# shamim-hussain/egt

Hardware: AMD Instinct MI355X
Metric: graphs/sec EGT fwd+bwd, ZINC-500K padded N=64 (higher is better)
Workload: dtype f32; 1 GPU; zinc500k_n64: attention-block stack (h,e,mask)->(h',e') x Ly, fwd+bwd + param grads; scope=stack, graphs_per_gpu=128, global_batch=128, N=64, Dh=64, De=64, H=8, d=8, Ly=10, parallelism=dp1, grad_allreduce_bytes=740480, backend=none (single process), flat_grad_adopted=True, flat_grad_bound=True, collective_in_graph=False

## Files before the change

### egt_amd/_lib.py

```python
from __future__ import annotations

import ctypes as C
import os

_HERE = os.path.dirname(os.path.abspath(__file__))
LIB_PATH = os.environ.get("EGT_AMD_LIB") or os.path.join(_HERE, "lib", "libegt_amd.so")

ABI_VERSION = 4
EGT_OK = 0
EGT_E_NULL, EGT_E_SHAPE, EGT_E_DTYPE, EGT_E_FLAGS, EGT_E_HIP, EGT_E_WORKSPACE, EGT_E_RCCL = -1, -2, -3, -4, -5, -6, -7
EGT_F32 = 0
EGT_BF16 = 1
F_EDGE_INPUT, F_GATE_INPUT, F_ATTN_MASK, F_SCALE_DEGREE = 0x001, 0x002, 0x004, 0x008
F_SCALER_LINEAR, F_TRAINING, F_CLIP = 0x010, 0x020, 0x040
ATTN_WS_SHARED = 0x1
EP_LAYERNORM, EP_GATES = 0x1, 0x2
ACT_NONE, ACT_LRELU, ACT_RELU, ACT_ELU = 0, 1, 2, 3
BF_GATE, BF_ATTN_MASK, BF_TRAINING, BF_CLIP, BF_NO_EDGE_LN, BF_SEED_DEVICE = 0x1, 0x2, 0x4, 0x8, 0x10, 0x20


class AttnDesc(C.Structure):
    _fields_ = [("B", C.c_int32), ("N", C.c_int32), ("H", C.c_int32), ("d", C.c_int32),
                ("dtype", C.c_int32), ("flags", C.c_uint32),
                ("clip_lo", C.c_float), ("clip_hi", C.c_float),
# ... 94 lines not shown
    "egt_dp_allreduce": (C.c_int, [_VP, C.c_size_t, C.c_int32, _VP]),
    "egt_dp_world": (C.c_int, []),
    "egt_dp_rank": (C.c_int, []),
    "egt_dp_finalize": (C.c_int, []),
    "egt_prof_enable": (C.c_int, [C.c_int]),
    "egt_prof_filter": (C.c_int, [C.c_char_p]),
    "egt_prof_stride": (C.c_int, [C.c_int]),
    "egt_prof_read": (C.c_int, [C.c_char_p, C.POINTER(C.c_int64), C.POINTER(C.c_double)]),
    "egt_prof_names": (C.c_int, [C.c_char_p, C.c_size_t]),
    "egt_prof_collect_graph": (C.c_int, [C.c_int]),
    "egt_prof_forget_graphs": (C.c_int, []),
}
_OPTIONAL_PROTOS = {
    "egt_block_supported": (C.c_int, [C.POINTER(BlockDesc)]),
    "egt_block_bwd_kernel": (C.c_char_p, [C.POINTER(BlockDesc)]),
    "egt_block_saved_bytes": (C.c_size_t, [C.POINTER(BlockDesc)]),
    "egt_block_workspace_bytes": (C.c_size_t, [C.POINTER(BlockDesc)]),
    "egt_block_fwd": (C.c_int, [C.POINTER(BlockDesc), C.POINTER(BlockParams)] + [_VP] * 10),
    "egt_block_bwd": (C.c_int, [C.POINTER(BlockDesc), C.POINTER(BlockParams)] + [_VP] * 10
                      + [C.POINTER(BlockParams)] + [_VP] * 2),
    "egt_stack_saved_bytes": (C.c_size_t, [C.POINTER(BlockDesc), C.c_int32]),
    "egt_stack_workspace_bytes": (C.c_size_t, [C.POINTER(BlockDesc), C.c_int32]),
    "egt_stack_fwd": (C.c_int, [C.POINTER(BlockDesc), C.c_int32, C.POINTER(BlockParams)] + [_VP] * 9),
    "egt_stack_bwd": (C.c_int, [C.POINTER(BlockDesc), C.c_int32, C.POINTER(BlockParams)] + [_VP] * 9
                      + [C.POINTER(BlockParams)] + [_VP] * 2),
    "egt_pair_supported": (C.c_int, [C.POINTER(BlockDesc)]),
    "egt_pair_workspace_bytes": (C.c_size_t, [C.POINTER(BlockDesc)]),
    "egt_pair_fwd": (C.c_int, [C.POINTER(BlockDesc), C.POINTER(BlockParams)] + [_VP] * 8),
    "egt_pair_bwd": (C.c_int, [C.POINTER(BlockDesc), C.POINTER(BlockParams)] + [_VP] * 9
                     + [C.POINTER(BlockParams)] + [_VP] * 2),
# ... 49 lines not shown
```

### egt_amd/csrc/egt_block.hip

```cpp
#include "egt_common.h"

#include <stdlib.h>
#include <string.h>
#include <vector>

#include "egt_block.h"
#include "egt_tile.h"

#include "egt_block_dev.h"
#include "egt_dma.h"

#include "egt_block_fwd.h"
#include "egt_block_bwd.h"



struct EgtBlockEnv {
  bool no_narrow_fwd, no_narrow_bwd;
  int bwd_mm;
  int bwd_tl, fwd_rows;
  int nrw_fwd_waves, nrw_bwd_waves, nrw_fwd_half;
};
static bool env_flag_raw(const char* name) {
  const char* v = getenv(name);
// ... 56 lines not shown

struct BlockPlan {
  bool ml;
  bool full;
  FwdKernel fwd;
  EgtLaunch fl;
  int fwd_nw;
  bool fwd_half;
  bool kvl;
  bool epi_ok;
  int RGF;
  BwdKernel bwd;
  EgtLaunch bl;
  int bwd_nw;
  int mm;
  int TL, NLR, nwg_bwd, EP;
  size_t v_att, stats, qkvp, pw_sv, wfrag_sv, saved_total;
  size_t dvp, dqp, dkvp, dqp_sz, dkvp_sz, common_total;
  size_t pw, epart, spart, sbo, wpart, ered, dqkv, dhbuf, layer_total;
};

template <int DE>
static BlockPlan plan_for(const egt_block_desc* d, bool ml) {
  using GG = Geo<DE>;
  const EgtBlockEnv& E = block_env();
  const int B = d->B, N = d->N, cus = egt_device_cus();
  const int groups = (N + BWD_TL - 1) / BWD_TL;
  BlockPlan P{};
  P.ml = ml;
  P.full = (N % 16) == 0;
// ... 29 lines not shown
  P.epi_ok = P.fwd != FwdKernel::tile || P.kvl;

  if (E.bwd_tl >= 4 && E.bwd_tl <= BWD_TL) P.TL = E.bwd_tl;
  else if (DE != 8) {
    const int g = tg > groups ? tg : groups;
    P.TL = (N + g - 1) / g;
  } else if (B * groups <= cus) {
    P.TL = BWD_TL;
    if (N > 8)
      for (int tl = 8; tl < BWD_TL; ++tl)
        if (B * ((N + tl - 1) / tl) <= cus) { P.TL = tl; break; }
  } else P.TL = (N + groups - 1) / groups;
  P.NLR = (N + P.TL - 1) / P.TL;
  P.nwg_bwd = B * P.NLR;
  P.EP = GG::EP;
  if (DE == 8 && !ml && !E.no_narrow_bwd) {
    P.bwd = BwdKernel::narrow;
    P.bwd_nw = E.nrw_bwd_waves == 8 || (E.nrw_bwd_waves != 4 && P.nwg_bwd <= cus && N >= 64) ? 8 : 4;
    P.bl = {P.nwg_bwd, 64 * P.bwd_nw, egt_narrow_bwd_lds(P.bwd_nw)};
  } else if (DE <= 16 && !ml) {
    constexpr int PWR = V4R_RR * (2 * GG::TILE_FLOATS + 256 + 192);
    P.bwd = BwdKernel::v4r;
    P.bl = {P.nwg_bwd, 256,
            ((size_t)(4 * PWR > BWD_PRO_WS ? 4 * PWR : BWD_PRO_WS) + (size_t)BWD_TL * QD_LD + 3 * GG::TILES * 256 + 3 * 2048 + 4) * 4};
  } else if (DE >= 32 && !ml && d->dtype != EGT_BF16) {
    P.bwd = BwdKernel::v5;
    P.mm = E.bwd_mm;
    P.bl = {P.nwg_bwd, 256, ((size_t)V5_AREA(DE) + (size_t)BWD_TL * QD_LD + 3 * ((GG::TILES + 1) / 2) * 512 + 4) * 4};
  } else {
    constexpr int PW = 3 * GG::TILE_FLOATS + 256 + 192;
    P.bwd = BwdKernel::v4;
    P.bl = {P.nwg_bwd, 256,
            ((size_t)(4 * PW > BWD_PRO_WS ? 4 * PW : BWD_PRO_WS) + (size_t)BWD_TL * QD_LD + 3 * ((GG::TILES + 1) / 2) * 512) * 4};
  }

  const size_t rows = (size_t)B * N;
  const int Dh = d->d * d->H;
  size_t o = 0;
  P.v_att = o; o += al(rows * Dh);
  P.stats = o; o += al(rows * BH * 4);
  P.qkvp = o; o += al(rows * QKVP);
  P.pw_sv = o; o += al((size_t)GG::DEP * 16 + 16);
// ... 36 lines not shown
  DISPATCH_BDE(d->De, return plan_for<DE>(d, ml));
}

static bool host_rand_mask(const egt_block_desc* d, const uint8_t* rm) {
  return rm && (d->flags & EGT_BF_TRAINING) && d->random_mask_prob > 0.0f;
}
static bool mask_tensor(const egt_block_desc* d, const uint8_t* rm) {
  return (d->flags & EGT_BF_ATTN_MASK) || host_rand_mask(d, rm);
}

static void bind_ws(const BlockPlan& P, BlockArgs& a, float* wc, float* wl, int parity = 0) {
  a.dvp = wc + P.dvp; a.dqp = wc + P.dqp + parity * P.dqp_sz; a.dkvp = wc + P.dkvp + parity * P.dkvp_sz;
  a.epart = wl + P.epart; a.spart = wl + P.spart; a.sbo = wl + P.sbo; a.wpart = wl + P.wpart;
  a.spart_n = a.sbo_n = a.B * ((a.N + NODE_RC - 1) / NODE_RC);
  a.ered = wl + P.ered; a.dqkv_sv = wl + P.dqkv;
  a.TL = P.TL; a.NLR = P.NLR; a.NQP = 1;
  a.xcd = 1;
}

extern "C" const char* egt_block_bwd_kernel(const egt_block_desc* d) {
  if (block_check(d, false)) return nullptr;
  return g_bwd_kernel_name[(int)plan_block(d, mask_tensor(d, nullptr)).bwd];
}

extern "C" size_t egt_block_saved_bytes(const egt_block_desc* d) {
  if (block_check(d, false)) return 0;
  return plan_block(d, mask_tensor(d, nullptr)).saved_total * sizeof(float);
}
extern "C" size_t egt_block_workspace_bytes(const egt_block_desc* d) {
  if (block_check(d, false)) return 0;
  const BlockPlan P = plan_block(d, mask_tensor(d, nullptr));
// ... 128 lines not shown
  static_assert(DE % 16 == 0 || DE == 8, "edge widths of the pair kernels");
  const bool pro = fuse;
  a.pro = 0;
  if (pro) {
    a.pro = top ? 1 : 2;
    a.sbo_n = P.nwg_bwd;
    if (!top) {
      a.up_h = above->h; a.up_nm_g = above->nm_g; a.up_Wqkv = above->Wqkv; a.up_wfrag = above->wfrag; a.up_dh_out = above->dh_out;
      a.up_dqp = above->dqp; a.up_dkvp = above->dkvp; a.up_dqkv_sv = above->dqkv_sv; a.up_spart = above->spart;
      above->spart_n = P.nwg_bwd;
    }
    if (a.prep) egt_node_launch_prep(&a, 1, st);
  } else if (top) {
    egt_node_launch_bwd(a, &a, false, st);
  }
  a.NQP = (a.N + 15) / 16;
  a.guard = 0;
  switch (P.bwd) {
    case BwdKernel::narrow: egt_narrow_launch_bwd(a, P.bwd_nw, P.bl, st); break;
    case BwdKernel::v4r:
      if constexpr (DE <= 16) {
        if (a.bf16) egt_launch_planned<k_block_bwd_v4r<DE, true, V4R_RR>>("k_block_bwd", P.bl, st, a);
        else egt_launch_planned<k_block_bwd_v4r<DE, false, V4R_RR>>("k_block_bwd", P.bl, st, a);
      }
      break;
    case BwdKernel::v5:
      if constexpr (DE >= 32) launch_v5<DE>(a, P, st);
      break;
    case BwdKernel::v4: if (a.bf16) launch_v4<DE, true>(a, P, st); else launch_v4<DE, false>(a, P, st); break;
  }
  if (!pro) egt_node_launch_bwd(a, below, true, st);
// ... 183 lines not shown
```

### egt_amd/csrc/egt_block_bwd.h

```cpp
#pragma once
#ifndef EGT_NT_BWD_E
#define EGT_NT_BWD_E true
#endif
#ifndef EGT_NT_BWD_DY
#define EGT_NT_BWD_DY false
#endif
#ifndef EGT_NT_BWD_ST
#define EGT_NT_BWD_ST false
#endif

template <int DE, bool ML, bool BF, bool RAG>
__global__ void __launch_bounds__(256, 2) k_block_bwd_v4(BlockArgs a) {
  seed_from_device(a);
  using G = Geo<DE>;
  typedef typename EdgeT<BF>::type ET;
  const ET* e_in = reinterpret_cast<const ET*>(a.e);
  ET* e_o = reinterpret_cast<ET*>(a.e_out);
  const ET* dey_in = reinterpret_cast<const ET*>(a.de_out);
  ET* dex_o = reinterpret_cast<ET*>(a.de);
  (void)e_in; (void)e_o; (void)dey_in; (void)dex_o;
  extern __shared__ __attribute__((aligned(16))) float sm[];
  const int lane = threadIdx.x & 63, wave = threadIdx.x >> 6;
  const int p = lane & 15, q = lane >> 4;
  const int N = a.N, TL = a.TL;
// ... 261 lines not shown
  if (p == 0) {
#pragma unroll
    for (int r = 0; r < 4; ++r) ep[G::DEP * 16 + 4 * q + r] = ssum[r];
  }
  __syncthreads();
  float* out = a.epart + (size_t)wg * G::EP;
  for (int i = threadIdx.x; i < G::EP; i += 256)
    out[i] = (sm[i] + sm[G::EP + i]) + (sm[2 * G::EP + i] + sm[3 * G::EP + i]);
}

#ifndef V5_BALANCE
#define V5_BALANCE 1
#endif
#define V5_AREA(DE_) ((4 * (3 * Geo<DE_>::TILE_FLOATS + 448) > 4 * Geo<DE_>::TILE_FLOATS + BWD_PRO_WS) \
                          ? 4 * (3 * Geo<DE_>::TILE_FLOATS + 448) : 4 * Geo<DE_>::TILE_FLOATS + BWD_PRO_WS)
template <int DE, int MM, bool RAG>
__global__ void __launch_bounds__(256, 2) k_block_bwd_v5(BlockArgs a) {
  seed_from_device(a);
#define PSTAMP(i) do {} while (0)
  constexpr bool SPLIT = MM == EGT_MM_BF16X3;
  constexpr int NS = (Geo<DE>::TILES + 1) / 2;
  (void)SPLIT; (void)NS;
  using G = Geo<DE>;
  const float* e_in = a.e;
  const float* dey_in = a.de_out;
  float* dex_o = a.de;
  extern __shared__ __attribute__((aligned(16))) float sm[];
  const int lane = threadIdx.x & 63, wave = __builtin_amdgcn_readfirstlane(threadIdx.x >> 6);
  const int p = lane & 15, q = lane >> 4;
  const int N = a.N, TL = a.TL;
// ... 15 lines not shown
  static_assert(4 * PW == 4 * G::TILE_FLOATS + 4 * PW2 && AREA >= 4 * PW && AREA >= 4 * G::TILE_FLOATS + BWD_PRO_WS, "tile area");
  float* pro_ws = sm + 4 * G::TILE_FLOATS;
  float* qd = sm + AREA;
  float* wsA = qd + TL * QD_LD;
  float* wsB = wsA + WSLAB;
  float* wsD = wsB + WSLAB;
  volatile int* pflag = reinterpret_cast<volatile int*>(wsD + WSLAB);
  if (threadIdx.x < 4) pflag[threadIdx.x] = 0;
  const unsigned et_lds = __builtin_amdgcn_readfirstlane((unsigned)(size_t)et0);
  const unsigned off0 = dma_lane_offset<DE>(lane);
  const int ntile = RAG ? (N + 15) / 16 : N / 16;
  const bool balance = RAG && V5_BALANCE && ntile >= 3 && (ntile & 3) != 0;
  const int T_ = ntile * nl;
  const int t0 = balance ? (wave * T_) >> 2 : 0, t1 = balance ? ((wave + 1) * T_) >> 2 : 0;
  const bool have = balance ? t1 > t0 : wave < ntile;
  const int mt_first = balance ? t0 / nl : wave, mt_last = balance ? (t1 - 1) / nl : ntile - 1, mt_step = balance ? 1 : 4;
  const int r0_first = balance ? t0 - mt_first * nl : 0;
  float Kf[16], Vf[16];
  int kmv = 1;
#define V5_TILE_START(MT_, ROW_)                                                                                    \
  do {                                                                                                              \
    const int m0_ = (MT_) * 16, kv_ = RAG ? min(16, N - m0_) : 16;                                                  \
    if (RAG && kv_ < 16) tile_dma_ragged<DE>(et_lds, e_in + (((size_t)b * N + l_begin + (ROW_)) * N + m0_) * DE, lane, kv_); \
    else tile_dma<DE, EGT_NT_BWD_E>(et_lds, e_in + (((size_t)b * N + l_begin + (ROW_)) * N + m0_) * DE, off0);      \
    const size_t rowm_ = (size_t)b * N + (RAG ? min(m0_ + p, N - 1) : m0_ + p);                                     \
    const float4* kp_ = reinterpret_cast<const float4*>(a.qkvp + rowm_ * QKVP + 64 + q * 16);                       \
    const float4* vp_ = reinterpret_cast<const float4*>(a.qkvp + rowm_ * QKVP + 128 + q * 16);                      \
    _Pragma("unroll") for (int i = 0; i < 4; ++i) {                                                                 \
      const float4 kv4 = kp_[i], vv4 = vp_[i];                                                                      \
      Kf[4*i] = kv4.x; Kf[4*i+1] = kv4.y; Kf[4*i+2] = kv4.z; Kf[4*i+3] = kv4.w;                                     \
// ... 99 lines not shown
    float dKa[16], dVa[16];
#pragma unroll
    for (int i = 0; i < 16; ++i) { dKa[i] = 0.f; dVa[i] = 0.f; }
    asm volatile("" : "+v"(kmv));
    const float kadd = kmv == 0 ? -EGT_NEG : 0.0f;
    const int l_first = l_begin + r0, l_stop = l_begin + r1;
    for (int l = l_first; l < l_stop; ++l) {
      const int li = l - l_begin;
      const int lj = l - l_first;
      const size_t rowl = (size_t)b * N + l;
      const size_t pair0 = rowl * N + m0;
      float* et = et0 + (lj & 1) * estr;
      MaskRegs mr{make_float2(1.f, 1.f), 0};
      TileRegs<DE> td;
      tile_gload<DE, EGT_NT_BWD_DY>(td, dey_in + pair0 * DE, lane, kv);
      if (lj == 0) vm_wait<(G::NF4 + 63) / 64>(); else vm_wait<2 * ((G::NF4 + 63) / 64) + 1>();
      SCHED_FENCE();
      float rstd;
      v4f acc = {c2r[0], c2r[1], c2r[2], c2r[3]};
      {
        float4 x[G::TILES];
#pragma unroll
        for (int t = 0; t < G::TILES; ++t) x[t] = frag_read<DE>(et, p, q, t);
        rstd = ln_frags<DE>(x, q, a.ln_eps, (a.flags & EGT_BF_NO_EDGE_LN) == 0);
        if constexpr (MM != 0) {
#pragma unroll
          for (int t = 0; t < G::TILES; ++t) frag_write<DE>(et, p, q, t, x[t]);
          v4f xv[G::TILES];
          Bf8 xh[NS], xl[NS];
#pragma unroll
          for (int t = 0; t < G::TILES; ++t) xv[t] = (v4f){x[t].x, x[t].y, x[t].z, x[t].w};
// ... 102 lines not shown
      {
        const float* qr = qd + li * QD_LD;
        const float4* qp = reinterpret_cast<const float4*>(qr + q * 16);
        const float4* dp = reinterpret_cast<const float4*>(qr + 64 + q * 16);
        float dq[16];
#pragma unroll
        for (int i = 0; i < 4; ++i) {
          const float4 u = qp[i], v = dp[i];
          dKa[4*i]   = fmaf(dA[0], u.x, dKa[4*i]);   dKa[4*i+1] = fmaf(dA[1], u.y, dKa[4*i+1]);
          dKa[4*i+2] = fmaf(dA[0], u.z, dKa[4*i+2]); dKa[4*i+3] = fmaf(dA[1], u.w, dKa[4*i+3]);
          dVa[4*i]   = fmaf(at[0], v.x, dVa[4*i]);   dVa[4*i+1] = fmaf(at[1], v.y, dVa[4*i+1]);
          dVa[4*i+2] = fmaf(at[0], v.z, dVa[4*i+2]); dVa[4*i+3] = fmaf(at[1], v.w, dVa[4*i+3]);
        }
#pragma unroll
        for (int k = 0; k < 8; ++k) { dq[2 * k] = dA[0] * Kf[2 * k]; dq[2 * k + 1] = dA[1] * Kf[2 * k + 1]; }
        a.dqp[(((size_t)b * ntile + mt) * N + l) * 64 + lane] = reduce16_keep_own(dq, p);
      }
      SCHED_FENCE();
      if (!(a.guard & 1))
      {
        float bT[4], bR[4];
#pragma unroll
        for (int s = 0; s < 4; ++s) {
          bT[s] = sc1[(q + 4 * s) * 16 + p];
          bR[s] = (p < 9) ? sc2[(q + 4 * s) * 12 + p] : 0.f;
        }
        {
          const int lb = 64 * q + 4 * ((p >> 2) ^ q) + (p & 3);
          const float* eb = et + lb;
          const float* db = dt + lb;
#pragma unroll
// ... 93 lines not shown
#pragma unroll
  for (int r = 0; r < 4; ++r) ssum[r] = row_sum16(ssum[r]);
  __syncthreads();
  float* ep = sm + wave * G::EP;
#pragma unroll
  for (int t = 0; t < G::TILES; ++t)
#pragma unroll
    for (int r = 0; r < 4; ++r) {
      ep[(16 * t + 4 * q + r) * 16 + p] = accT[t][r];
      ep[G::DEP * 16 + 16 + (16 * t + 4 * q + r) * 16 + p] = accR[t][r];
    }
  if (p == 0) {
#pragma unroll
    for (int r = 0; r < 4; ++r) ep[G::DEP * 16 + 4 * q + r] = ssum[r];
  }
  __syncthreads();
  float* out = a.epart + (size_t)wg * G::EP;
  for (int i = threadIdx.x; i < G::EP; i += 256)
    out[i] = (sm[i] + sm[G::EP + i]) + (sm[2 * G::EP + i] + sm[3 * G::EP + i]);
}

template <int DE, bool BF, int R>
__global__ void __launch_bounds__(256, 2) k_block_bwd_v4r(BlockArgs a) {
  seed_from_device(a);
  using G = Geo<DE>;
  typedef typename EdgeT<BF>::type ET;
  const ET* e_in = reinterpret_cast<const ET*>(a.e);
  const ET* dey_in = reinterpret_cast<const ET*>(a.de_out);
  ET* dex_o = reinterpret_cast<ET*>(a.de);
  extern __shared__ __attribute__((aligned(16))) float sm[];
  const int lane = threadIdx.x & 63, wave = threadIdx.x >> 6;
  const int p = lane & 15, q = lane >> 4;
  const int N = a.N, TL = a.TL;
  const int wg = a.xcd ? egt_xcd_remap(blockIdx.x, gridDim.x) : (int)blockIdx.x;
// ... 321 lines not shown
```

### egt_amd/csrc/egt_node.hip

```cpp
#include <stdlib.h>

#include "egt_block.h"

#define LDP 4

__device__ __forceinline__ float sum16(float v) { return row_sum16(v); }

__device__ __forceinline__ v4f mm_xw(const float* xs, int ld, const float* W, int ldw,
                                     int K, int p, int q, bool colok, v4f acc) {
#pragma unroll 4
  for (int t = 0; t < K; t += 4) {
    const float bv = colok ? W[(size_t)(t + q) * ldw + p] : 0.f;
    acc = MFMA(xs[p * ld + t + q], bv, acc);
  }
  return acc;
}
__device__ __forceinline__ v4f mm_xwt(const float* xs, int ld, const float* W, int ldw,
                                      int K, int p, int q, bool colok, v4f acc) {
#pragma unroll 4
  for (int t = 0; t < K; t += 4) {
    const float bv = colok ? W[(size_t)p * ldw + t + q] : 0.f;
    acc = MFMA(xs[p * ld + t + q], bv, acc);
  }
  return acc;
// ... 309 lines not shown
            a.h_out[o] = acc[r] + a.h[o];
          }
        }
      }
    }
  }
}

struct NodeBwdArgs {
  const float *wq_a, *wo_a;
  int wq_al, wo_al;
  const float *dv_Wo, *dv_v_att, *dv_dh_src;
  float *dv_stats, *dv_dvp, *dv_sbo;
};

template <bool PRE, bool DV, int NP>
__global__ void __launch_bounds__(512, 2) k_node_bwd(BlockArgs a, NodeBwdArgs x) {
  extern __shared__ __attribute__((aligned(16))) float sm[];
  const int NCH = (a.N + NODE_RC - 1) / NODE_RC;
  if ((int)blockIdx.x == a.B * NCH) { prep_device(a, sm); return; }
  const int Dh = a.Dh, N = a.N, b = blockIdx.x / NCH, chunk = blockIdx.x % NCH, t = threadIdx.x, D3 = 3 * Dh;
  const int ld = Dh + LDP, ld3 = D3 + LDP, SP = D3 + 2 * Dh;
  const int lane = t & 63, wave = __builtin_amdgcn_readfirstlane(t >> 6), p = lane & 15, q = lane >> 4, NW = blockDim.x >> 6;
  float* xs = sm;
  float* dls = xs + NODE_RC * ld;
  float* dhs = dls + NODE_RC * ld;
  float* vs = dhs + NODE_RC * ld;
  float* rs = vs + NODE_RC * ld;
  float* dlp = rs + NODE_RC;
  float* wo = dlp + 4 * NODE_RC * 8;
  float* dqs = wo + Dh * ld;
// ... 27 lines not shown
    }
    const int U = nrp * 48;
#pragma unroll
    for (int u = 0; u < 3; ++u) {
      const int i = t + u * 512, r = i / 48, pos4 = (i % 48) * 4, sx = pos4 >> 6;
      const bool ok = i < U && r < nr;
      const int rc = ok ? r : 0;
      float4 acc4 = make_float4(0.f, 0.f, 0.f, 0.f);
      const int np = sx == 0 ? a.NQP : a.NLR;
      const float* base = sx == 0 ? a.dqp + ((size_t)b * a.NQP * N + r0 + rc) * 64 + pos4
                                  : a.dkvp + (((size_t)b * a.NLR * N + r0 + rc) * 2 + (sx - 1)) * 64 + (pos4 & 63);
      const size_t pstride = sx == 0 ? (size_t)N * 64 : (size_t)N * 128;
      if (NP > 0) {
#pragma unroll
        for (int pi = 0; pi < NP; ++pi) {
          const float4 w = *reinterpret_cast<const float4*>(base + pi * pstride);
          acc4.x += w.x; acc4.y += w.y; acc4.z += w.z; acc4.w += w.w;
        }
      } else {
        const int npmax = max(a.NQP, a.NLR);
#pragma unroll 4
        for (int pi = 0; pi < npmax; ++pi) {
          const float4 w = *reinterpret_cast<const float4*>(base + min(pi, np - 1) * pstride);
          const float f = pi < np ? 1.0f : 0.0f;
          acc4.x = fmaf(w.x, f, acc4.x); acc4.y = fmaf(w.y, f, acc4.y);
          acc4.z = fmaf(w.z, f, acc4.z); acc4.w = fmaf(w.w, f, acc4.w);
        }
      }
      gq[u] = sel4(ok, acc4);
    }
  } else {
    stg_issue_rows(sX, x.dv_dh_src + row0 * Dh, Dh, nr, nrp);
// ... 137 lines not shown
    __syncthreads();
    for (int i = t; i < nr * 8; i += blockDim.x) {
      float dl = 0.f;
      for (int it = 0; it < nit; ++it) dl += dlp[it * NODE_RC * 8 + i];
      x.dv_stats[(row0 * BH + i) * 4 + 2] = dl;
    }
    if (a.DK < 8) {
      for (int i = t; i < nr * 64; i += blockDim.x)
        if ((((i & 63) >> 1) & 7) >= a.DK) x.dv_dvp[row0 * 64 + i] = 0.f;
    }
  }
}

#define WG_ROWS 128
struct WGradLayer { const float *h, *nm_g, *nm_b, *dqkv, *v_att, *dh_out; float* part; };
struct WGradArgs { WGradLayer L[64]; int rows, Dh, rows_per_wg; float ln_eps; };

template <bool D64>
__global__ void __launch_bounds__(512, 4) k_node_wgrads(WGradArgs wa) {
  extern __shared__ __attribute__((aligned(16))) float sm[];
  const WGradLayer L = wa.L[blockIdx.y];
  const int Dh = D64 ? 64 : wa.Dh, D3 = 3 * Dh, t = threadIdx.x;
  const int ld = Dh + 16, ld3 = D3 + 16;
  const int lane = t & 63, wave = __builtin_amdgcn_readfirstlane(t >> 6), p = lane & 15, q = lane >> 4, NW = blockDim.x >> 6;
  float* xs = sm;
  float* vs = xs + 32 * ld;
  float* ds = vs + 32 * ld;
  float* dqs = ds + 32 * ld;
  const int nkt = (Dh + 15) / 16, nct = (D3 + 15) / 16;
  const int kt = wave >> 1, ct0 = (wave & 1) * 6, co0 = (wave & 1) * 2;
  v4f accW[6], accO[2];
#pragma unroll
  for (int j = 0; j < 6; ++j) accW[j] = (v4f){0.f, 0.f, 0.f, 0.f};
#pragma unroll
  for (int j = 0; j < 2; ++j) accO[j] = (v4f){0.f, 0.f, 0.f, 0.f};
  const int rbeg = blockIdx.x * wa.rows_per_wg, rend = min(wa.rows, rbeg + wa.rows_per_wg);
  const int w4 = Dh >> 2, w43 = 3 * w4;
  const bool xok = t < 32 * w4;
  const int xr = xok ? t / w4 : 0, xc = xok ? t % w4 : 0;
  int qr[3], qc[3];
  bool qok[3];
#pragma unroll
  for (int u = 0; u < 3; ++u) {
    const int i = t + 512 * u;
    qok[u] = i < 32 * w43;
    qr[u] = qok[u] ? i / w43 : 0;
    qc[u] = qok[u] ? i % w43 : 0;
  }
  float gam[4], bet[4];
#pragma unroll
  for (int i = 0; i < 4; ++i) {
    const int c = p + 16 * i;
    gam[i] = c < Dh ? L.nm_g[c] : 0.f;
    bet[i] = c < Dh ? L.nm_b[c] : 0.f;
  }
  float4 gam4 = make_float4(0.f, 0.f, 0.f, 0.f), bet4 = gam4;
  if (D64) {
    gam4 = make_float4(L.nm_g[xc * 4], L.nm_g[xc * 4 + 1], L.nm_g[xc * 4 + 2], L.nm_g[xc * 4 + 3]);
    bet4 = make_float4(L.nm_b[xc * 4], L.nm_b[xc * 4 + 1], L.nm_b[xc * 4 + 2], L.nm_b[xc * 4 + 3]);
  }
  float4 ph, pv, pd, pq[3];
#define WG_LOAD(R0)                                                                              \
  do {                                                                                           \
// ... 49 lines not shown
#pragma unroll
      for (int rr = 0; rr < 32; rr += 4) {
        const float av = xs[(rr + q) * ld + kt * 16 + p];
        const float vv = vs[(rr + q) * ld + kt * 16 + p];
        const float* dr = dqs + (rr + q) * ld3 + p;
        const float* dd = ds + (rr + q) * ld + p;
#pragma unroll
        for (int j = 0; j < 6; ++j)
          if (D64 || ct0 + j < nct) accW[j] = MFMA(av, dr[(ct0 + j) * 16], accW[j]);
#pragma unroll
        for (int j = 0; j < 2; ++j)
          if (D64 || co0 + j < nkt) accO[j] = MFMA(vv, dd[(co0 + j) * 16], accO[j]);
      }
    }
  }
  float* part = L.part + (size_t)blockIdx.x * (Dh * D3 + Dh * Dh);
  if (kt < nkt) {
#pragma unroll
    for (int j = 0; j < 6; ++j) {
      const int c = (ct0 + j) * 16 + p;
      if (ct0 + j < nct) {
#pragma unroll
        for (int r = 0; r < 4; ++r) {
          const int kk = kt * 16 + 4 * q + r;
          if (kk < Dh && c < D3) part[kk * D3 + c] = accW[j][r];
        }
      }
    }
#pragma unroll
    for (int j = 0; j < 2; ++j) {
      const int c = (co0 + j) * 16 + p;
      if (co0 + j < nkt) {
#pragma unroll
        for (int r = 0; r < 4; ++r) {
          const int i = kt * 16 + 4 * q + r;
          if (i < Dh && c < Dh) part[Dh * D3 + i * Dh + c] = accO[j][r];
        }
      }
    }
  }
}

struct SumSeg { const float* src; float* dst; int n, np, stride, blk0; };
#define SUM_MAX_SEG 77
struct SumArgs { SumSeg seg[SUM_MAX_SEG]; int nseg; };

#define SUM_G 8
#define SUM_U 8
__global__ void __launch_bounds__(32 * SUM_G) k_sum_segments(SumArgs s) {
  __shared__ float red[SUM_G][32];
  int lo = 0, hi = s.nseg - 1;
  while (lo < hi) {
    const int mid = (lo + hi + 1) >> 1;
    if (s.seg[mid].blk0 <= (int)blockIdx.x) lo = mid; else hi = mid - 1;
  }
// ... 138 lines not shown

void egt_node_launch_bwd(BlockArgs& a, const BlockArgs* dv_layer, bool do_pre, hipStream_t st) {
  NodeBwdArgs x{};
  auto down16 = [](const float* p) { return reinterpret_cast<const float*>(reinterpret_cast<uintptr_t>(p) & ~(uintptr_t)15); };
  x.wq_a = down16(a.Wqkv); x.wq_al = x.wq_a == a.Wqkv;
  if (dv_layer) {
    x.wo_a = down16(dv_layer->Wo); x.wo_al = x.wo_a == dv_layer->Wo;
    x.dv_Wo = dv_layer->Wo; x.dv_v_att = dv_layer->v_att; x.dv_dh_src = a.dh_out;
    x.dv_stats = dv_layer->stats; x.dv_dvp = dv_layer->dvp; x.dv_sbo = dv_layer->sbo;
  }
  const int Dh = a.Dh, ld = Dh + LDP, ld3 = 3 * Dh + LDP;
  size_t lds = ((size_t)4 * NODE_RC * ld + NODE_RC + 4 * NODE_RC * 8 + (size_t)Dh * ld) * 4;
  if (do_pre) lds += ((size_t)NODE_RC * ld3 + (size_t)Dh * ld3) * 4;
  const bool prep = !do_pre && a.prep;
  const dim3 grid(a.B * node_chunks(a) + (prep ? 1 : 0));
#define NODE_BWD(PRE_, DV_, NP_, NAME)                                                                     \
  do {                                                                                                 \
    EGT_MAX_LDS_ONCE(k_node_bwd<PRE_, DV_, NP_>); \
    EGT_LAUNCH(NAME, (k_node_bwd<PRE_, DV_, NP_>), grid, dim3(512), lds, st, a, x);                    \
  } while (0)
  const bool np4 = a.NQP == 4 && a.NLR == 4;
  if (!do_pre) NODE_BWD(false, true, 0, "k_node_bwd_top");
  else if (dv_layer) { if (np4) NODE_BWD(true, true, 4, "k_node_bwd"); else NODE_BWD(true, true, 0, "k_node_bwd"); }
  else { if (np4) NODE_BWD(true, false, 4, "k_node_bwd"); else NODE_BWD(true, false, 0, "k_node_bwd"); }
#undef NODE_BWD
}

static int wgrad_rows_per_wg(int rows, int layers) {
  int per_layer = (2 * egt_device_cus()) / (layers > 0 ? layers : 1);
  if (per_layer < 1) per_layer = 1;
  const int r = (((rows + per_layer - 1) / per_layer + 31) / 32) * 32;
  return r < WG_ROWS ? WG_ROWS : r;
}
int egt_node_wgrad_chunks(int rows, int layers) { const int r = wgrad_rows_per_wg(rows, layers); return (rows + r - 1) / r; }

void egt_node_launch_wgrads(BlockArgs* as, int n, hipStream_t st) {
  WGradArgs wa{};
  const BlockArgs& a0 = as[0];
  wa.rows = a0.B * a0.N; wa.Dh = a0.Dh; wa.ln_eps = a0.ln_eps; wa.rows_per_wg = wgrad_rows_per_wg(wa.rows, n);
  for (int l = 0; l < n; ++l) {
    const BlockArgs& a = as[l];
    wa.L[l] = WGradLayer{a.h, a.nm_g, a.nm_b, a.dqkv_sv, a.v_att, a.dh_out, a.wpart};
  }
  const int Dh = a0.Dh;
  const size_t lds = ((size_t)3 * 32 * (Dh + 16) + (size_t)32 * (3 * Dh + 16)) * 4;
  const dim3 grid(egt_node_wgrad_chunks(wa.rows, n), n);
  for (int l = 0; l < n; ++l) as[l].wpart_n = (int)grid.x;
  if (Dh == 64) EGT_LAUNCH("k_node_wgrads", k_node_wgrads<true>, grid, dim3(512), lds, st, wa);
  else EGT_LAUNCH("k_node_wgrads", k_node_wgrads<false>, grid, dim3(512), lds, st, wa);
}

void egt_node_launch_prep(BlockArgs* as, int n, hipStream_t st) {
  for (int l0 = 0; l0 < n; l0 += PREP_MAX_LAYERS) {
    const int nl = n - l0 < PREP_MAX_LAYERS ? n - l0 : PREP_MAX_LAYERS;
    PrepArgs pa{};
    pa.De = as[0].De; pa.Dh = as[0].Dh; pa.flags = as[0].flags;
    for (int l = 0; l < nl; ++l) {
      const BlockArgs& a = as[l0 + l];
      pa.L[l] = PrepLayer{a.ne_g, a.ne_b, a.Wg, a.bg, a.We, a.be, a.pw, a.Wqkv, a.Wo, a.wfrag};
    }
    EGT_LAUNCH("k_edge_prep", k_edge_prep, dim3(nl), dim3(256), 0, st, pa);
  }
// ... 40 lines not shown
```

### include/egt_amd.h

```cpp
#ifndef EGT_AMD_H_
#define EGT_AMD_H_

#include <stddef.h>
#include <stdint.h>

#ifdef __cplusplus
extern "C" {
#endif

#define EGT_ABI_VERSION 4

#define EGT_OK 0
#define EGT_E_NULL (-1)
#define EGT_E_SHAPE (-2)
#define EGT_E_DTYPE (-3)
#define EGT_E_FLAGS (-4)
#define EGT_E_HIP (-5)
#define EGT_E_WORKSPACE (-6)
#define EGT_E_RCCL (-7)

#define EGT_F32 0
#define EGT_BF16 1

#define EGT_F_EDGE_INPUT 0x001u
// ... 123 lines not shown
  const void* attention_gates_bias;
  const void* dense_edge_b_kernel;
  const void* dense_edge_b_bias;
  const void* norm_mha_gamma;
  const void* norm_mha_beta;
  const void* dense_qkv_kernel;
  const void* dense_qkv_bias;
  const void* dense_mha_kernel;
  const void* dense_mha_bias;
  const void* dense_edge_r_kernel;
  const void* dense_edge_r_bias;
} egt_block_params;

int egt_block_supported(const egt_block_desc* desc);
const char* egt_block_bwd_kernel(const egt_block_desc* desc);
size_t egt_block_saved_bytes(const egt_block_desc* desc);
size_t egt_block_workspace_bytes(const egt_block_desc* desc);

int egt_block_fwd(const egt_block_desc* desc, const egt_block_params* params,
                  const void* h, const void* e, const uint8_t* key_mask,
                  const void* attn_mask, const uint8_t* rand_mask, void* h_out,
                  void* e_out, void* saved, void* workspace, void* stream);

int egt_block_bwd(const egt_block_desc* desc, const egt_block_params* params,
                  const void* h, const void* e, const uint8_t* key_mask,
                  const void* attn_mask, const uint8_t* rand_mask,
                  const void* saved, const void* d_h_out, const void* d_e_out,
                  void* d_h, void* d_e, const egt_block_params* grads,
                  void* workspace, void* stream);

// ... 103 lines not shown
```

Before: 79630 graphs/s.

## Accumulate dQ partials in registers for v5 bwd and flatten node wgrad grid

In the v5 block backward kernel, when N is a multiple of 16 the per-tile dQ partials are kept in registers, reduced across the four waves through LDS, and written once per workgroup as a single slab (NQP=1) instead of one partial per query tile. The node backward kernel gains a Q1 variant that reads only the one valid dQ partial. Separately, the node weight-gradient kernel now runs over a flat, balanced 1D grid of 32-row steps spread across layers to fill about two workgroups per CU, with a fallback to the per-layer layout. This cuts dQ partial traffic and reduce work and should improve wgrad load balance, in exchange for more register pressure and extra LDS staging in the v5 kernel.

```diff
diff --git a/egt_amd/_lib.py b/egt_amd/_lib.py
--- a/egt_amd/_lib.py
+++ b/egt_amd/_lib.py
@@ -132,6 +132,7 @@
 _OPTIONAL_PROTOS = {
     "egt_block_supported": (C.c_int, [C.POINTER(BlockDesc)]),
     "egt_block_bwd_kernel": (C.c_char_p, [C.POINTER(BlockDesc)]),
+    "egt_node_wgrad_plan": (C.c_int, [C.c_int32, C.c_int32, C.POINTER(C.c_int32), C.POINTER(C.c_int32)]),
     "egt_block_saved_bytes": (C.c_size_t, [C.POINTER(BlockDesc)]),
     "egt_block_workspace_bytes": (C.c_size_t, [C.POINTER(BlockDesc)]),
     "egt_block_fwd": (C.c_int, [C.POINTER(BlockDesc), C.POINTER(BlockParams)] + [_VP] * 10),
diff --git a/egt_amd/csrc/egt_block.hip b/egt_amd/csrc/egt_block.hip
--- a/egt_amd/csrc/egt_block.hip
+++ b/egt_amd/csrc/egt_block.hip
@@ -94,6 +94,7 @@
   EgtLaunch bl;
   int bwd_nw;
   int mm;
+  int nqp;
   int TL, NLR, nwg_bwd, EP;
   size_t v_att, stats, qkvp, pw_sv, wfrag_sv, saved_total;
   size_t dvp, dqp, dkvp, dqp_sz, dkvp_sz, common_total;
@@ -153,6 +154,7 @@
   P.NLR = (N + P.TL - 1) / P.TL;
   P.nwg_bwd = B * P.NLR;
   P.EP = GG::EP;
+  P.nqp = (N + 15) / 16;
   if (DE == 8 && !ml && !E.no_narrow_bwd) {
     P.bwd = BwdKernel::narrow;
     P.bwd_nw = E.nrw_bwd_waves == 8 || (E.nrw_bwd_waves != 4 && P.nwg_bwd <= cus && N >= 64) ? 8 : 4;
@@ -165,6 +167,7 @@
   } else if (DE >= 32 && !ml && d->dtype != EGT_BF16) {
     P.bwd = BwdKernel::v5;
     P.mm = E.bwd_mm;
+    if (v5_dq_slab(N)) P.nqp = 1;
     P.bl = {P.nwg_bwd, 256, ((size_t)V5_AREA(DE) + (size_t)BWD_TL * QD_LD + 3 * ((GG::TILES + 1) / 2) * 512 + 4) * 4};
   } else {
     constexpr int PW = 3 * GG::TILE_FLOATS + 256 + 192;
@@ -231,7 +234,7 @@
   a.epart = wl + P.epart; a.spart = wl + P.spart; a.sbo = wl + P.sbo; a.wpart = wl + P.wpart;
   a.spart_n = a.sbo_n = a.B * ((a.N + NODE_RC - 1) / NODE_RC);
   a.ered = wl + P.ered; a.dqkv_sv = wl + P.dqkv;
-  a.TL = P.TL; a.NLR = P.NLR; a.NQP = 1;
+  a.TL = P.TL; a.NLR = P.NLR; a.NQP = P.nqp;
   a.xcd = 1;
 }
 
@@ -390,7 +393,6 @@
   } else if (top) {
     egt_node_launch_bwd(a, &a, false, st);
   }
-  a.NQP = (a.N + 15) / 16;
   a.guard = 0;
   switch (P.bwd) {
     case BwdKernel::narrow: egt_narrow_launch_bwd(a, P.bwd_nw, P.bl, st); break;
diff --git a/egt_amd/csrc/egt_block_bwd.h b/egt_amd/csrc/egt_block_bwd.h
--- a/egt_amd/csrc/egt_block_bwd.h
+++ b/egt_amd/csrc/egt_block_bwd.h
@@ -299,6 +299,8 @@
 #endif
 #define V5_AREA(DE_) ((4 * (3 * Geo<DE_>::TILE_FLOATS + 448) > 4 * Geo<DE_>::TILE_FLOATS + BWD_PRO_WS) \
                           ? 4 * (3 * Geo<DE_>::TILE_FLOATS + 448) : 4 * Geo<DE_>::TILE_FLOATS + BWD_PRO_WS)
+#define V5_DQ_SLAB_FLOATS (4 * BWD_TL * 64)
+inline bool v5_dq_slab(int N) { return (N % 16) == 0; }
 template <int DE, int MM, bool RAG>
 __global__ void __launch_bounds__(256, 2) k_block_bwd_v5(BlockArgs a) {
   seed_from_device(a);
@@ -344,6 +346,9 @@
   const int T_ = ntile * nl;
   const int t0 = balance ? (wave * T_) >> 2 : 0, t1 = balance ? ((wave + 1) * T_) >> 2 : 0;
   const bool have = balance ? t1 > t0 : wave < ntile;
+  constexpr bool dq_slab = !RAG;
+  typedef float v16f __attribute__((ext_vector_type(BWD_TL)));
+  v16f dqr = 0.f;
   const int mt_first = balance ? t0 / nl : wave, mt_last = balance ? (t1 - 1) / nl : ntile - 1, mt_step = balance ? 1 : 4;
   const int r0_first = balance ? t0 - mt_first * nl : 0;
   float Kf[16], Vf[16];
@@ -473,7 +478,9 @@
       MaskRegs mr{make_float2(1.f, 1.f), 0};
       TileRegs<DE> td;
       tile_gload<DE, EGT_NT_BWD_DY>(td, dey_in + pair0 * DE, lane, kv);
-      if (lj == 0) vm_wait<(G::NF4 + 63) / 64>(); else vm_wait<2 * ((G::NF4 + 63) / 64) + 1>();
+      if (lj == 0) vm_wait<(G::NF4 + 63) / 64>();
+      else if (dq_slab) vm_wait<2 * ((G::NF4 + 63) / 64)>();
+      else vm_wait<2 * ((G::NF4 + 63) / 64) + 1>();
       SCHED_FENCE();
       float rstd;
       v4f acc = {c2r[0], c2r[1], c2r[2], c2r[3]};
@@ -606,7 +613,9 @@
         }
 #pragma unroll
         for (int k = 0; k < 8; ++k) { dq[2 * k] = dA[0] * Kf[2 * k]; dq[2 * k + 1] = dA[1] * Kf[2 * k + 1]; }
-        a.dqp[(((size_t)b * ntile + mt) * N + l) * 64 + lane] = reduce16_keep_own(dq, p);
+        const float dqv = reduce16_keep_own(dq, p);
+        if (dq_slab) dqr[__builtin_amdgcn_readfirstlane(li)] += dqv;
+        else a.dqp[(((size_t)b * ntile + mt) * N + l) * 64 + lane] = dqv;
       }
       SCHED_FENCE();
       if (!(a.guard & 1))
@@ -730,10 +739,27 @@
 #pragma unroll
     for (int r = 0; r < 4; ++r) ep[G::DEP * 16 + 4 * q + r] = ssum[r];
   }
+  static_assert(4 * G::EP + V5_DQ_SLAB_FLOATS <= AREA && (4 * G::EP) % 4 == 0, "dQ slab in the tile area");
+  float* dqs = sm + 4 * G::EP;
+  if (dq_slab) {
+#pragma unroll
+    for (int i = 0; i < BWD_TL; ++i) dqs[(wave * BWD_TL + i) * 64 + lane] = dqr[i];
+  }
   __syncthreads();
   float* out = a.epart + (size_t)wg * G::EP;
   for (int i = threadIdx.x; i < G::EP; i += 256)
     out[i] = (sm[i] + sm[G::EP + i]) + (sm[2 * G::EP + i] + sm[3 * G::EP + i]);
+  if (dq_slab) {
+    float4* dqo = reinterpret_cast<float4*>(a.dqp + ((size_t)b * N + l_begin) * 64);
+    for (int i = threadIdx.x; i < nl * 16; i += 256) {
+      const float4 s0 = *reinterpret_cast<const float4*>(dqs + 4 * i);
+      const float4 s1 = *reinterpret_cast<const float4*>(dqs + BWD_TL * 64 + 4 * i);
+      const float4 s2 = *reinterpret_cast<const float4*>(dqs + 2 * BWD_TL * 64 + 4 * i);
+      const float4 s3 = *reinterpret_cast<const float4*>(dqs + 3 * BWD_TL * 64 + 4 * i);
+      dqo[i] = make_float4(((s0.x + s1.x) + s2.x) + s3.x, ((s0.y + s1.y) + s2.y) + s3.y,
+                           ((s0.z + s1.z) + s2.z) + s3.z, ((s0.w + s1.w) + s2.w) + s3.w);
+    }
+  }
 }
 
 template <int DE, bool BF, int R>
diff --git a/egt_amd/csrc/egt_node.hip b/egt_amd/csrc/egt_node.hip
--- a/egt_amd/csrc/egt_node.hip
+++ b/egt_amd/csrc/egt_node.hip
@@ -347,7 +347,7 @@
   float *dv_stats, *dv_dvp, *dv_sbo;
 };
 
-template <bool PRE, bool DV, int NP>
+template <bool PRE, bool DV, int NP, bool Q1 = false>
 __global__ void __launch_bounds__(512, 2) k_node_bwd(BlockArgs a, NodeBwdArgs x) {
   extern __shared__ __attribute__((aligned(16))) float sm[];
   const int NCH = (a.N + NODE_RC - 1) / NODE_RC;
@@ -405,8 +405,9 @@
       if (NP > 0) {
 #pragma unroll
         for (int pi = 0; pi < NP; ++pi) {
-          const float4 w = *reinterpret_cast<const float4*>(base + pi * pstride);
-          acc4.x += w.x; acc4.y += w.y; acc4.z += w.z; acc4.w += w.w;
+          const bool in = !Q1 || pi == 0 || sx != 0;
+          const float4 w = *reinterpret_cast<const float4*>(base + (in ? pi : 0) * pstride);
+          acc4.x += in ? w.x : 0.f; acc4.y += in ? w.y : 0.f; acc4.z += in ? w.z : 0.f; acc4.w += in ? w.w : 0.f;
         }
       } else {
         const int npmax = max(a.NQP, a.NLR);
@@ -574,13 +575,23 @@
 
 #define WG_ROWS 128
 struct WGradLayer { const float *h, *nm_g, *nm_b, *dqkv, *v_att, *dh_out; float* part; };
-struct WGradArgs { WGradLayer L[64]; int rows, Dh, rows_per_wg; float ln_eps; };
+struct WGradArgs { WGradLayer L[64]; int rows, Dh, spl, spw, wpl, steps; float ln_eps; };
 
 template <bool D64>
 __global__ void __launch_bounds__(512, 4) k_node_wgrads(WGradArgs wa) {
   extern __shared__ __attribute__((aligned(16))) float sm[];
-  const WGradLayer L = wa.L[blockIdx.y];
-  const int Dh = D64 ? 64 : wa.Dh, D3 = 3 * Dh, t = threadIdx.x;
+  const int wgi = blockIdx.x;
+  const int s0 = wa.wpl ? (wgi / wa.wpl) * wa.spl + (wgi % wa.wpl) * wa.spw : wgi * wa.spw;
+  const int s1 = min(wa.wpl ? (wgi / wa.wpl + 1) * wa.spl : wa.steps, s0 + wa.spw);
+  for (int sg = s0; sg < s1;) {
+  const int layer = sg / wa.spl, sb = layer * wa.spl, se = min(s1, sb + wa.spl);
+  const WGradLayer L = wa.L[layer];
+  const int slot = wa.wpl ? (sg - sb) / wa.spw : wgi - sb / wa.spw;
+  const int rbeg = (sg - sb) * 32, rend = min(wa.rows, (se - sb) * 32);
+  sg = se;
+  int t = threadIdx.x;
+  asm volatile("" : "+v"(t));
+  const int Dh = D64 ? 64 : wa.Dh, D3 = 3 * Dh;
   const int ld = Dh + 16, ld3 = D3 + 16;
   const int lane = t & 63, wave = __builtin_amdgcn_readfirstlane(t >> 6), p = lane & 15, q = lane >> 4, NW = blockDim.x >> 6;
   float* xs = sm;
@@ -589,12 +600,6 @@
   float* dqs = ds + 32 * ld;
   const int nkt = (Dh + 15) / 16, nct = (D3 + 15) / 16;
   const int kt = wave >> 1, ct0 = (wave & 1) * 6, co0 = (wave & 1) * 2;
-  v4f accW[6], accO[2];
-#pragma unroll
-  for (int j = 0; j < 6; ++j) accW[j] = (v4f){0.f, 0.f, 0.f, 0.f};
-#pragma unroll
-  for (int j = 0; j < 2; ++j) accO[j] = (v4f){0.f, 0.f, 0.f, 0.f};
-  const int rbeg = blockIdx.x * wa.rows_per_wg, rend = min(wa.rows, rbeg + wa.rows_per_wg);
   const int w4 = Dh >> 2, w43 = 3 * w4;
   const bool xok = t < 32 * w4;
   const int xr = xok ? t / w4 : 0, xc = xok ? t % w4 : 0;
@@ -607,6 +612,11 @@
     qr[u] = qok[u] ? i / w43 : 0;
     qc[u] = qok[u] ? i % w43 : 0;
   }
+  v4f accW[6], accO[2];
+#pragma unroll
+  for (int j = 0; j < 6; ++j) accW[j] = (v4f){0.f, 0.f, 0.f, 0.f};
+#pragma unroll
+  for (int j = 0; j < 2; ++j) accO[j] = (v4f){0.f, 0.f, 0.f, 0.f};
   float gam[4], bet[4];
 #pragma unroll
   for (int i = 0; i < 4; ++i) {
@@ -686,7 +696,7 @@
       }
     }
   }
-  float* part = L.part + (size_t)blockIdx.x * (Dh * D3 + Dh * Dh);
+  float* part = L.part + (size_t)slot * (Dh * D3 + Dh * Dh);
   if (kt < nkt) {
 #pragma unroll
     for (int j = 0; j < 6; ++j) {
@@ -711,6 +721,8 @@
       }
     }
   }
+  }
+#undef WG_LOAD
 }
 
 struct SumSeg { const float* src; float* dst; int n, np, stride, blk0; };
@@ -879,15 +891,22 @@
   if (do_pre) lds += ((size_t)NODE_RC * ld3 + (size_t)Dh * ld3) * 4;
   const bool prep = !do_pre && a.prep;
   const dim3 grid(a.B * node_chunks(a) + (prep ? 1 : 0));
-#define NODE_BWD(PRE_, DV_, NP_, NAME)                                                                     \
+#define NODE_BWD(PRE_, DV_, NP_, Q1_, NAME)                                                                \
   do {                                                                                                 \
-    EGT_MAX_LDS_ONCE(k_node_bwd<PRE_, DV_, NP_>); \
-    EGT_LAUNCH(NAME, (k_node_bwd<PRE_, DV_, NP_>), grid, dim3(512), lds, st, a, x);                    \
+    EGT_MAX_LDS_ONCE(k_node_bwd<PRE_, DV_, NP_, Q1_>); \
+    EGT_LAUNCH(NAME, (k_node_bwd<PRE_, DV_, NP_, Q1_>), grid, dim3(512), lds, st, a, x);               \
   } while (0)
-  const bool np4 = a.NQP == 4 && a.NLR == 4;
-  if (!do_pre) NODE_BWD(false, true, 0, "k_node_bwd_top");
-  else if (dv_layer) { if (np4) NODE_BWD(true, true, 4, "k_node_bwd"); else NODE_BWD(true, true, 0, "k_node_bwd"); }
-  else { if (np4) NODE_BWD(true, false, 4, "k_node_bwd"); else NODE_BWD(true, false, 0, "k_node_bwd"); }
+#define NODE_BWD_NP(PRE_, DV_)                                                                         \
+  do {                                                                                                 \
+    if (np4 && a.NQP == 1) NODE_BWD(PRE_, DV_, 4, true, "k_node_bwd");                                 \
+    else if (np4) NODE_BWD(PRE_, DV_, 4, false, "k_node_bwd");                                         \
+    else NODE_BWD(PRE_, DV_, 0, false, "k_node_bwd");                                                  \
+  } while (0)
+  const bool np4 = a.NLR == 4 && (a.NQP == 4 || a.NQP == 1);
+  if (!do_pre) NODE_BWD(false, true, 0, false, "k_node_bwd_top");
+  else if (dv_layer) NODE_BWD_NP(true, true);
+  else NODE_BWD_NP(true, false);
+#undef NODE_BWD_NP
 #undef NODE_BWD
 }
 
@@ -899,18 +918,53 @@
 }
 int egt_node_wgrad_chunks(int rows, int layers) { const int r = wgrad_rows_per_wg(rows, layers); return (rows + r - 1) / r; }
 
+#ifndef EGT_WGRAD_FLAT
+#define EGT_WGRAD_FLAT 1
+#endif
+struct WGradPlan { int spl, spw, wpl, nwg; };
+static int wgrad_layer_parts(const WGradPlan& W, int l) {
+  if (W.wpl) return W.wpl;
+  return ((l + 1) * W.spl - 1) / W.spw - (l * W.spl) / W.spw + 1;
+}
+static WGradPlan wgrad_plan(int rows, int layers) {
+  WGradPlan W{};
+  W.spl = (rows + 31) / 32;
+  const int steps = W.spl * layers, slots = 2 * egt_device_cus(), reserved = egt_node_wgrad_chunks(rows, 1);
+  W.spw = (steps + slots - 1) / slots;
+  if (W.spw < WG_ROWS / 32) W.spw = WG_ROWS / 32;
+  W.wpl = 0;
+  W.nwg = (steps + W.spw - 1) / W.spw;
+  bool fits = EGT_WGRAD_FLAT != 0;
+  for (int l = 0; l < layers; ++l) fits = fits && wgrad_layer_parts(W, l) <= reserved;
+  if (!fits) {
+    W.spw = wgrad_rows_per_wg(rows, layers) / 32;
+    W.wpl = (W.spl + W.spw - 1) / W.spw;
+    W.nwg = W.wpl * layers;
+  }
+  return W;
+}
+extern "C" int egt_node_wgrad_plan(int32_t rows, int32_t layers, int32_t* out, int32_t* parts) {
+  if (rows < 1 || layers < 1 || layers > 64 || !out || !parts) return -1;
+  const WGradPlan W = wgrad_plan(rows, layers);
+  out[0] = W.spl; out[1] = W.spw; out[2] = W.wpl; out[3] = W.nwg; out[4] = egt_node_wgrad_chunks(rows, 1);
+  for (int l = 0; l < layers; ++l) parts[l] = wgrad_layer_parts(W, l);
+  return 0;
+}
+
 void egt_node_launch_wgrads(BlockArgs* as, int n, hipStream_t st) {
   WGradArgs wa{};
   const BlockArgs& a0 = as[0];
-  wa.rows = a0.B * a0.N; wa.Dh = a0.Dh; wa.ln_eps = a0.ln_eps; wa.rows_per_wg = wgrad_rows_per_wg(wa.rows, n);
+  const WGradPlan W = wgrad_plan(a0.B * a0.N, n);
+  wa.rows = a0.B * a0.N; wa.Dh = a0.Dh; wa.ln_eps = a0.ln_eps;
+  wa.spl = W.spl; wa.spw = W.spw; wa.wpl = W.wpl; wa.steps = W.spl * n;
   for (int l = 0; l < n; ++l) {
     const BlockArgs& a = as[l];
     wa.L[l] = WGradLayer{a.h, a.nm_g, a.nm_b, a.dqkv_sv, a.v_att, a.dh_out, a.wpart};
   }
   const int Dh = a0.Dh;
   const size_t lds = ((size_t)3 * 32 * (Dh + 16) + (size_t)32 * (3 * Dh + 16)) * 4;
-  const dim3 grid(egt_node_wgrad_chunks(wa.rows, n), n);
-  for (int l = 0; l < n; ++l) as[l].wpart_n = (int)grid.x;
+  const dim3 grid(W.nwg);
+  for (int l = 0; l < n; ++l) as[l].wpart_n = wgrad_layer_parts(W, l);
   if (Dh == 64) EGT_LAUNCH("k_node_wgrads", k_node_wgrads<true>, grid, dim3(512), lds, st, wa);
   else EGT_LAUNCH("k_node_wgrads", k_node_wgrads<false>, grid, dim3(512), lds, st, wa);
 }
diff --git a/include/egt_amd.h b/include/egt_amd.h
--- a/include/egt_amd.h
+++ b/include/egt_amd.h
@@ -161,6 +161,7 @@
 
 int egt_block_supported(const egt_block_desc* desc);
 const char* egt_block_bwd_kernel(const egt_block_desc* desc);
+int egt_node_wgrad_plan(int32_t rows, int32_t layers, int32_t* out, int32_t* parts);
 size_t egt_block_saved_bytes(const egt_block_desc* desc);
 size_t egt_block_workspace_bytes(const egt_block_desc* desc);
 
```

Result: no change. 79770 graphs/s (median of 6 runs) (+0.2%).
